# aimi-lab/robust-pose-estimator

Hardware: AMD Instinct MI355X
Metric: stereo-pair pose solves/sec (640x512, 8 solver iters) (higher is better)
Workload: dtype f32 (RAFT / geometry) + f64 (SE(3) solve), as the reference; 1 GPU; PoseNet.infer, 640x512 stereo frame pairs, 16 per GPU per step (RAFT batch 32), 12 GRU iters, lbfgs x8 SE(3) solve, weight heads on; frames_per_gpu=16, height=512, width=640, raft_iters=12, solver=lbfgs, solver_iters=8, parallelism=frames sharded x1

## Files before the change

robust-pose-estimator_amd/csrc/conv.hip:

```cpp
#include "conv_host.h"
#include "conv_igemm.h"
#include <type_traits>

template <int KW, int WM, bool ENC, int T, bool VERT, bool S2>
__global__ __launch_bounds__(256, 3) void k_conv_igemm(ConvP P) {
    constexpr int WN = 4 / WM, WT = 32 * T, BM = WT * WM, BN = WT * WN, PW = VERT ? 0 : KW / 2;
    constexpr int VTX = 16, VTY = 8, VROWS = VTY + KW - 1;
    constexpr int KS = 20;
    constexpr int NLA = BM / 64;
    constexpr int NLB = VERT ? (VROWS * VTX / 4 * CK + 255) / 256 : S2 ? BN / 32 : BN / 64;
    __shared__ __attribute__((aligned(16))) float As[2][BM][KS];
    __shared__ __attribute__((aligned(16))) float Bs[2][VERT ? VROWS * VTX : S2 ? 2 * BN + 8 : BN + 8][KS];
    const int bz = blockIdx.z, m0 = blockIdx.y * BM, n0 = blockIdx.x * BN;
    const int vtiles_x = (P.W + VTX - 1) / VTX;
    const int vx0 = VERT ? (blockIdx.x % vtiles_x) * VTX : 0, vy0 = VERT ? (blockIdx.x / vtiles_x) * VTY : 0;
    const int tid = threadIdx.x, lane = tid & 63, wv = tid >> 6, l31 = lane & 31, lh = lane >> 5;
    const int wm = wv / WN, wn = wv % WN;
    const int W = P.W, hw = P.hw, ph = P.kh / 2;
    __shared__ __attribute__((aligned(8))) float sbt[ENC ? BM : 1][2];
    if (ENC && tid < BM) {
        const int co = m0 + tid;
        sbt[tid][0] = (P.scale && co < P.cout) ? P.scale[co] : 1.0f;
        sbt[tid][1] = (P.bias && co < P.cout) ? P.bias[co] : 0.0f;
    }
// ... 304 lines not shown
#pragma unroll
                for (int r = 0; r < 4; ++r) {
                    const int row = row0 + r + 8 * (rb >> 2), co = m0 + row;
                    const bool cok = co < P.cout;
                    const float2 s2 = *(const float2*)&sbt[row][0];
                    sc[r] = s2.x; bi[r] = s2.y;
#pragma unroll
                    for (int j = 0; j < T; ++j) {
                        const int px = n0 + wn * WT + j * 32 + l31;
                        ok[j][r] = cok && px < hw;
                        e[j][r] = ok[j][r] ? (size_t)co * hw + px : 0;
                    }
                }
                if (EXTRA) {
#pragma unroll
                    for (int j = 0; j < T; ++j)
#pragma unroll
                        for (int r = 0; r < 4; ++r) {
                            rv[j][r] = resb ? resb[e[j][r]] : 0.0f;
                            av[j][r] = addb ? addb[e[j][r]] : 0.0f;
                        }
                }
#pragma unroll
                for (int r = 0; r < 4; ++r) {
                    float vv[T];
#pragma unroll
                    for (int j = 0; j < T; ++j) {
                        if (EXTRA) { float v = acc[i][j][rb + r] * sc[r]; v += av[j][r]; v += bi[r]; vv[j] = v; }
                        else vv[j] = fmaf(acc[i][j][rb + r], sc[r], bi[r]);
                    }
                    float piv[NS], ssum[NS], ssq[NS];
                    if (STATS) {
#pragma unroll
                        for (int s2 = 0; s2 < NS; ++s2) {
                            const int vb = __builtin_bit_cast(int, vv[S2 ? s2 : 0]);
                            piv[s2] = __builtin_bit_cast(float, lh ? __builtin_amdgcn_readlane(vb, 32) : __builtin_amdgcn_readlane(vb, 0));
                            ssum[s2] = 0.0f; ssq[s2] = 0.0f;
                        }
                    }
#pragma unroll
                    for (int j = 0; j < T; ++j) {
                        float v = vv[j];
                        if (STATS) { const float dv = ok[j][r] ? v - piv[S2 ? j : 0] : 0.0f; ssum[S2 ? j : 0] += dv; ssq[S2 ? j : 0] = fmaf(dv, dv, ssq[S2 ? j : 0]); }
                        if (relu) v = v < 0.0f ? 0.0f : v;
                        if (EXTRA && resb) { v = rv[j][r] + v; v = v < 0.0f ? 0.0f : v; }
                        if (ok[j][r]) { outb[e[j][r]] = v; if (EXTRA && out2b) out2b[e[j][r]] = v; }
                    }
                    if (STATS) {
                        const int row = row0 + r + 8 * (rb >> 2);
#pragma unroll
                        for (int s2 = 0; s2 < NS; ++s2) {
                            const float a = half_wave_sum(ssum[s2]), q = half_wave_sum(ssq[s2]);
                            float* rd = red + ((wn * NS + s2) * BM + row) * 3;
                            if (l31 == 31) { rd[0] = a; rd[1] = q; rd[2] = piv[s2]; }
                        }
                    }
                }
            }
        }
    };
    {
        typedef std::integral_constant<bool, true> Yes; typedef std::integral_constant<bool, false> No;
        const bool extra = P.res || P.add || P.out2;
        if (P.stats) { if (extra) epilogue(Yes{}, Yes{}); else epilogue(Yes{}, No{}); }
        else { if (extra) epilogue(No{}, Yes{}); else epilogue(No{}, No{}); }
    }
    if (P.stats) {
        __syncthreads();
        if (S2) {
            const int nrec = (hw + 31) / 32;
            if (tid < BM && m0 + tid < P.cout) {
#pragma unroll
                for (int w2 = 0; w2 < WN; ++w2)
#pragma unroll
                    for (int s2 = 0; s2 < NS; ++s2) {
                        const int blk = (n0 + w2 * WT + s2 * 32) >> 5;
                        if (blk >= nrec) continue;
                        int nw = hw - blk * 32; nw = nw > 32 ? 32 : nw;
                        const float* rd = red + ((w2 * NS + s2) * BM + tid) * 3;
                        StatAcc A;
                        A.add_pivoted(nw, rd[0], rd[1], rd[2]);
                        float* st = P.stats + (((size_t)bz * P.cout + m0 + tid) * nrec + blk) * 3;
                        st[0] = (float)A.n; st[1] = (float)A.mean; st[2] = (float)A.m2;
                    }
            }
        } else if (tid < BM && m0 + tid < P.cout) {
            StatAcc A;
#pragma unroll
            for (int w2 = 0; w2 < WN; ++w2) {
                int nw = hw - (n0 + w2 * WT); nw = nw < 0 ? 0 : (nw > WT ? WT : nw);
                A.add_pivoted(nw, red[(w2 * BM + tid) * 3], red[(w2 * BM + tid) * 3 + 1], red[(w2 * BM + tid) * 3 + 2]);
            }
            float* st = P.stats + (((size_t)bz * P.cout + m0 + tid) * gridDim.x + blockIdx.x) * 3;
            st[0] = (float)A.n; st[1] = (float)A.mean; st[2] = (float)A.m2;
        }
    }
}

__device__ __forceinline__ void plane_moments(const float* __restrict__ partials, int tiles_signed, int C, int plane, int nthreads, double* sh, double& mean, double& var) {
    const int tiles = tiles_signed < 0 ? -tiles_signed : tiles_signed;
    const int ts = tiles_signed < 0 ? 3 * C : 3;
    const float* pp = tiles_signed < 0 ? partials + ((size_t)(plane / C) * tiles * C + (plane % C)) * 3 : partials + (size_t)plane * tiles * 3;
    double n = 0.0, a = 0.0;
    for (int i = threadIdx.x; i < tiles; i += nthreads) { n += (double)pp[(size_t)ts * i]; a += (double)pp[(size_t)ts * i] * (double)pp[(size_t)ts * i + 1]; }
    n = wave_sum(n); a = wave_sum(a);
    const int nw = nthreads >> 6, wv = threadIdx.x >> 6;
    if (nw > 1) {
        if ((threadIdx.x & 63) == 0) { sh[wv] = n; sh[4 + wv] = a; }
        __syncthreads();
        n = 0.0; a = 0.0;
        for (int w = 0; w < nw; ++w) { n += sh[w]; a += sh[4 + w]; }
        __syncthreads();
    }
    mean = a / n;
    double q = 0.0;
    for (int i = threadIdx.x; i < tiles; i += nthreads) { const double d = (double)pp[(size_t)ts * i + 1] - mean; q += (double)pp[(size_t)ts * i + 2] + (double)pp[(size_t)ts * i] * d * d; }
    q = wave_sum(q);
    if (nw > 1) {
        if ((threadIdx.x & 63) == 0) sh[wv] = q;
        __syncthreads();
        q = 0.0;
        for (int w = 0; w < nw; ++w) q += sh[w];
    }
    var = q / n;
    var = var < 0.0 ? 0.0 : var;
}

__global__ __launch_bounds__(256) void k_instnorm_finalize(const float* __restrict__ partials, int tiles, int C, int hw, float eps, float* __restrict__ mi) {
    const int plane = blockIdx.x;
    __shared__ double sh[8];
    double mean, var;
    plane_moments(partials, tiles, C, plane, 256, sh, mean, var);
    if (threadIdx.x == 0) { mi[(size_t)plane * 2] = (float)mean; mi[(size_t)plane * 2 + 1] = (float)(1.0 / sqrt(var + (double)eps)); }
    (void)hw;
}

__global__ __launch_bounds__(256) void k_instnorm_finalize_tm(const float* __restrict__ partials, int tiles, int C, float eps, float* __restrict__ mi) {
    const int b = blockIdx.y, cl = threadIdx.x & 3, sl = threadIdx.x >> 2, c = blockIdx.x * 4 + cl;
    __shared__ double sh[2][64][4];
    const bool ok = c < C;
    const float* pp = partials + ((size_t)b * tiles * C + (ok ? c : 0)) * 3;
    const size_t ts = (size_t)3 * C;
    auto tree = [&](double (*v)[4]) {
#pragma unroll
        for (int h = 32; h >= 1; h >>= 1) {
            __syncthreads();
            if (sl < h) v[sl][cl] += v[sl + h][cl];
        }
        __syncthreads();
    };
    constexpr int RMAX = 20;
    float rn[RMAX], rm[RMAX], rq[RMAX];
    const bool held = tiles <= 64 * RMAX;
    if (held) {
#pragma unroll
        for (int j = 0; j < RMAX; ++j) {
            const int t = sl + 64 * j;
            const float* r = pp + ts * (size_t)(t < tiles ? t : 0);
            const float v0 = r[0], v1 = r[1], v2 = r[2];
            rn[j] = t < tiles ? v0 : 0.0f; rm[j] = v1; rq[j] = v2;
        }
    }
    double n = 0.0, a = 0.0;
    if (held) {
#pragma unroll
        for (int j = 0; j < RMAX; ++j) if (sl + 64 * j < tiles) { const double nt = (double)rn[j]; n += nt; a += nt * (double)rm[j]; }
    } else {
        for (int t = sl; t < tiles; t += 64) { const double nt = (double)pp[ts * t]; n += nt; a += nt * (double)pp[ts * t + 1]; }
    }
    sh[0][sl][cl] = n; sh[1][sl][cl] = a;
    tree(sh[0]); tree(sh[1]);
    n = sh[0][0][cl]; a = sh[1][0][cl];
    const double mean = a / n;
    double q = 0.0;
    if (held) {
#pragma unroll
        for (int j = 0; j < RMAX; ++j) if (sl + 64 * j < tiles) { const double d = (double)rm[j] - mean; q += (double)rq[j] + (double)rn[j] * d * d; }
    } else {
        for (int t = sl; t < tiles; t += 64) { const double d = (double)pp[ts * t + 1] - mean; q += (double)pp[ts * t + 2] + (double)pp[ts * t] * d * d; }
    }
    __syncthreads();
    sh[0][sl][cl] = q;
    tree(sh[0]);
    if (sl == 0 && ok) {
        double var = sh[0][0][cl] / n;
        var = var < 0.0 ? 0.0 : var;
        float* o = mi + ((size_t)b * C + c) * 2;
        o[0] = (float)mean; o[1] = (float)(1.0 / sqrt(var + (double)eps));
    }
}

__global__ __launch_bounds__(256) void k_instnorm_apply(const float* __restrict__ x, const float* __restrict__ partials, int tiles, int C, int hw,
                                                        float eps, int relu, const float* __restrict__ residual, const float* __restrict__ res_mi,
                                                        float* __restrict__ out, int split) {
    const int plane = blockIdx.x / split, part = blockIdx.x % split;
    __shared__ double sh[8];
    float mean, inv;
    if (tiles == 0) { mean = partials[(size_t)plane * 2]; inv = partials[(size_t)plane * 2 + 1]; }
    else {
        double dmean, dvar;
        plane_moments(partials, tiles, C, plane, 256, sh, dmean, dvar);
        mean = (float)dmean; inv = (float)(1.0 / sqrt(dvar + (double)eps));
    }
    const float4* xp = (const float4*)(x + (size_t)plane * hw);
    const float4* rp = residual ? (const float4*)(residual + (size_t)plane * hw) : nullptr;
    float4* op = (float4*)(out + (size_t)plane * hw);
    const bool rnorm = res_mi != nullptr;
    const float rmean = rnorm ? res_mi[(size_t)plane * 2] : 0.0f, rinv = rnorm ? res_mi[(size_t)plane * 2 + 1] : 1.0f;
    const bool yrelu = relu & 1, rrelu = !(relu & 2);
    auto fin = [&](float v, float r) -> float {
        float y = (v - mean) * inv;
        if (yrelu) y = y < 0.0f ? 0.0f : y;
        if (rp) {
            if (rnorm) { r = (r - rmean) * rinv; if (rrelu) r = r < 0.0f ? 0.0f : r; }
            y = r + y; y = y < 0.0f ? 0.0f : y;
        }
        return y;
    };
#ifndef INA_UNROLL
#define INA_UNROLL 4
#endif
#ifndef INA_NT
#define INA_NT 3
#endif
    typedef float f4 __attribute__((ext_vector_type(4)));
    const int n4all = hw >> 2;
    const int per = ((n4all + split - 1) / split + 3) & ~3;
    const int n4 = (part + 1) * per < n4all ? (part + 1) * per : n4all;
    int i = part * per + threadIdx.x;
    for (; i + (INA_UNROLL - 1) * (int)blockDim.x < n4; i += INA_UNROLL * blockDim.x) {
        f4 v[INA_UNROLL], r[INA_UNROLL];
#pragma unroll
        for (int u = 0; u < INA_UNROLL; ++u) {
            const int j = i + u * blockDim.x;
            v[u] = INA_NT ? __builtin_nontemporal_load((const f4*)xp + j) : ((const f4*)xp)[j];
            r[u] = rp ? (INA_NT ? __builtin_nontemporal_load((const f4*)rp + j) : ((const f4*)rp)[j]) : (f4){0.f, 0.f, 0.f, 0.f};
        }
#pragma unroll
        for (int u = 0; u < INA_UNROLL; ++u) {
            const f4 o = {fin(v[u][0], r[u][0]), fin(v[u][1], r[u][1]), fin(v[u][2], r[u][2]), fin(v[u][3], r[u][3])};
            if (INA_NT & 2) __builtin_nontemporal_store(o, (f4*)op + i + u * blockDim.x); else ((f4*)op)[i + u * blockDim.x] = o;
        }
    }
    for (; i < n4; i += blockDim.x) {
        const float4 v = xp[i];
        const float4 r = rp ? rp[i] : make_float4(0.f, 0.f, 0.f, 0.f);
        op[i] = make_float4(fin(v.x, r.x), fin(v.y, r.y), fin(v.z, r.z), fin(v.w, r.w));
    }
}

__global__ void k_conv_pack(const float* __restrict__ w, float* __restrict__ wp, int cout, int cin, int kh, int kw, int coP,
                            long long total) {
    const long long e = (long long)blockIdx.x * blockDim.x + threadIdx.x;
    if (e >= total) return;
    const int ke = (int)(e & 3);
    const int co = (int)((e >> 2) % coP);
    const long long rest = (e >> 2) / coP;
    const int k4 = (int)(rest & 3);
    const long long s = rest >> 2;
    const int dx = (int)(s % kw), dy = (int)((s / kw) % kh), c = (int)(s / ((long long)kw * kh));
    const int ci = c * CK + 4 * k4 + ke;
    wp[e] = (co < cout && ci < cin) ? w[(((size_t)co * cin + ci) * kh + dy) * kw + dx] : 0.0f;
}

static inline bool conv_wide(int cout) { return (cout % 128) != 0 && (cout % 128) <= 96; }
static inline bool conv_s2_small(int cout, int hw_out, int b) { return (long long)ceil_div(hw_out, 128) * ceil_div(cout, 128) * b < 512; }

extern "C" size_t rpe_conv_packed_floats(int cout, int cin, int kh, int kw) {
    if (cout <= 0 || cin <= 0 || kh <= 0 || kw <= 0) return 0;
    return ((size_t)((cin + CK - 1) / CK) * kh * kw + 1) * CK * round_up(cout, 128);
}

extern "C" int rpe_conv_pack(const float* weight, int cout, int cin, int kh, int kw, float* packed, void* stream) {
    if (kh <= 0 || kw <= 0) return RPE_E_BADARG;
    return launch_pack(k_conv_pack, weight, packed, cout, cin, 1, (long long)rpe_conv_packed_floats(cout, cin, kh, kw), stream, kh, kw, round_up(cout, 128));
}

static_assert(sizeof(rpe_conv_desc) == 200, "rpe_conv_desc layout is part of the ABI (ctypes mirror in _lib.py)");

static int conv_fused(const rpe_conv_desc* d, void* stream, bool m96) {
    if (!conv_desc_present(d)) return RPE_E_BADARG;
    if (d->kh < 1 || !(d->kh & 1) || (d->kw != 1 && d->kw != 3 && d->kw != 5)) return RPE_E_UNSUPPORTED;
    if ((d->w & 3) || !aligned16(d->x, d->x_batch_stride)) return RPE_E_UNSUPPORTED;
    if (d->mode < RPE_CONV_LINEAR || d->mode > RPE_CONV_TANH) return RPE_E_BADARG;
    if (d->mode == RPE_CONV_TANH && (!conv_no_encoder_epilogue(d) || !stride_is_1(d) ||
                                     ((d->cout % 64) != 0 && (d->cout % 64) <= 32 && d->kw == 3))) return RPE_E_UNSUPPORTED;
    if (!conv_gate_args_ok(d)) return RPE_E_BADARG;
    if ((d->mode == RPE_CONV_GATE_ZR || d->mode == RPE_CONV_GATE_H) && (d->scale || d->residual || d->stats)) return RPE_E_BADARG;
    const int stride = d->stride ? d->stride : 1;
    if (stride != 1 && stride != 2) return RPE_E_UNSUPPORTED;
    if (d->pre_norm && (stride != 1 || d->kw != 3 || d->mode > RPE_CONV_RELU)) return RPE_E_UNSUPPORTED;
    if (stride == 2 && ((d->h & 1) || (d->w & 1) || d->mode > RPE_CONV_RELU || !((d->kh == 3 && d->kw == 3) || (d->kh == 1 && d->kw == 1))))
        return RPE_E_UNSUPPORTED;
    ConvP P;
    fill_common(P, d, round_up(d->cout, 128)); fill_gate(P, d); fill_encoder(P, d);
    P.kh = d->kh; P.Hin = d->h; P.Win = d->w; P.H = d->h / stride; P.W = d->w / stride; P.hw = P.H * P.W;
    P.h = d->hidden; P.hbs = d->hidden_batch_stride;
    hipStream_t s = (hipStream_t)stream;
    if (stride == 2) {
        const int t128 = ceil_div(P.hw, 128), t64 = ceil_div(P.hw, 64);
        const bool small = conv_s2_small(d->cout, P.hw, d->b);
        if (d->stats && d->stats_tiles != 0 && d->stats_tiles != ceil_div(P.hw, 32)) return RPE_E_BADARG;
        if (m96 && d->kw == 3 && d->cout == 96 && !d->residual && !d->add && !d->out2) return conv_s2_m96_launch(P, d->b, s);
        if (small) {
            dim3 g2(t64, ceil_div(d->cout, 64), d->b);
            if (d->kw == 3) hipLaunchKernelGGL((k_conv_igemm<3, 2, true, 1, false, true>), g2, dim3(256), 0, s, P);
            else hipLaunchKernelGGL((k_conv_igemm<1, 2, true, 1, false, true>), g2, dim3(256), 0, s, P);
            return rpe_check_launch();
        }
        dim3 g2(t128, ceil_div(d->cout, 128), d->b);
        if (d->kw == 3) hipLaunchKernelGGL((k_conv_igemm<3, 2, true, 2, false, true>), g2, dim3(256), 0, s, P);
        else hipLaunchKernelGGL((k_conv_igemm<1, 2, true, 2, false, true>), g2, dim3(256), 0, s, P);
        return rpe_check_launch();
    }
    bool wide = conv_wide(d->cout);
    int BM = wide ? 64 : 128, BN = wide ? 256 : 128;
    const bool half_tile = (d->cout % 64) != 0 && (d->cout % 64) <= 32 && d->kw == 3 && d->mode <= RPE_CONV_RELU;
    const bool enc = d->scale || d->residual || d->stats || d->pre_norm || half_tile;
    const bool small = !enc && (long long)ceil_div(P.hw, BN) * ceil_div(d->cout, BM) * d->b < 512;
    if (small) { BM = 64; BN = 64; }
    dim3 grid(ceil_div(P.hw, BN), ceil_div(d->cout, BM), d->b), block(256);
#define LAUNCH(KW_, WM_, ENC_, T_) hipLaunchKernelGGL((k_conv_igemm<KW_, WM_, ENC_, T_, false, false>), grid, block, 0, s, P)
    if (enc) {
        if (d->kw != 3 || d->mode > RPE_CONV_RELU) return RPE_E_UNSUPPORTED;
        if (wide) LAUNCH(3, 1, true, 2); else LAUNCH(3, 2, true, 2);
    } else if (small) { if (d->kw == 1) LAUNCH(1, 2, false, 1); else if (d->kw == 3) LAUNCH(3, 2, false, 1); else LAUNCH(5, 2, false, 1); }
    else if (wide) { if (d->kw == 1) LAUNCH(1, 1, false, 2); else if (d->kw == 3) LAUNCH(3, 1, false, 2); else LAUNCH(5, 1, false, 2); }
    else if (d->kw == 1 && d->kh == 5) {
        dim3 vgrid(ceil_div(d->w, 16) * ceil_div(d->h, 8), grid.y, grid.z);
        hipLaunchKernelGGL((k_conv_igemm<5, 2, false, 2, true, false>), vgrid, block, 0, s, P);
    } else         { if (d->kw == 1) LAUNCH(1, 2, false, 2); else if (d->kw == 3) LAUNCH(3, 2, false, 2); else LAUNCH(5, 2, false, 2); }
#undef LAUNCH
    return rpe_check_launch();
}

extern "C" int rpe_conv_fused(const rpe_conv_desc* d, void* stream) { return conv_fused(d, stream, false); }
extern "C" int rpe_conv_fused_m96(const rpe_conv_desc* d, void* stream) { return conv_fused(d, stream, true); }

extern "C" int rpe_conv_stats_tiles(int cout, int h, int w, int stride) {
    if (cout <= 0 || h <= 0 || w <= 0 || (stride != 1 && stride != 2)) return 0;
    if (stride == 2) return ceil_div((int64_t)(h / 2) * (w / 2), 32);
    return ceil_div((int64_t)h * w, conv_wide(cout) ? 256 : 128);
}

extern "C" int rpe_conv_stats_tiles_batch(int cout, int h, int w, int stride, int b) {
    if (b <= 0) return 0;
    return rpe_conv_stats_tiles(cout, h, w, stride);
}

extern "C" int rpe_instnorm_apply_ex(const float* x, const float* partials, int tiles, int b, int c, int hw, float eps, int relu,
                                     const float* residual, const float* residual_mean_inv, float* out, void* stream) {
    if (!x || !partials || !out || b <= 0 || c <= 0 || hw <= 0 || (residual_mean_inv && !residual)) return RPE_E_BADARG;
    if ((hw & 3) || !aligned16(x, 0) || !aligned16(out, 0) || !aligned16(residual, 0)) return RPE_E_UNSUPPORTED;
    int split = 1;
#ifndef INA_MAXSPLIT
#define INA_MAXSPLIT 16
#endif
#ifndef INA_MINBYTES
#define INA_MINBYTES 16384
#endif
    if (tiles == 0) while (split < INA_MAXSPLIT && (long long)hw * 4 / (split * 2) >= INA_MINBYTES) split *= 2;
    hipLaunchKernelGGL(k_instnorm_apply, dim3(b * c * split), dim3(256), 0, (hipStream_t)stream, x, partials, tiles, c, hw, eps, relu, residual,
                       residual_mean_inv, out, split);
    return rpe_check_launch();
}

extern "C" int rpe_instnorm_apply(const float* x, const float* partials, int tiles, int b, int c, int hw, float eps, int relu,
                                  const float* residual, float* out, void* stream) {
    return rpe_instnorm_apply_ex(x, partials, tiles, b, c, hw, eps, relu, residual, nullptr, out, stream);
}

extern "C" int rpe_instnorm_finalize(const float* partials, int tiles, int b, int c, int hw, float eps, float* mean_inv, void* stream) {
    if (!partials || !mean_inv || tiles == 0 || b <= 0 || c <= 0 || hw <= 0) return RPE_E_BADARG;
    if (tiles < 0) hipLaunchKernelGGL(k_instnorm_finalize_tm, dim3(ceil_div(c, 4), b), dim3(256), 0, (hipStream_t)stream, partials, -tiles, c, eps, mean_inv);
    else hipLaunchKernelGGL(k_instnorm_finalize, dim3(b * c), dim3(256), 0, (hipStream_t)stream, partials, tiles, c, hw, eps, mean_inv);
    return rpe_check_launch();
}
```

robust-pose-estimator_amd/csrc/conv_igemm.h:

```cpp
#pragma once
#include "rpe_common.h"

typedef float f32x16 __attribute__((ext_vector_type(16)));
#define CK 16
#define SCHED_FENCE() __builtin_amdgcn_sched_barrier(0)

struct ConvP {
    const float* x; long long xbs;
    const float* wp;
    int cin, cout, coP, H, W, hw, kh;
    int Hin, Win;
    const float* bias;
    const float* add; long long abs_;
    int mode;
    float* out; long long obs;
    float* out2; long long o2bs;
    const float* h; long long hbs;
    const float* z; long long zbs;
    int cgate;
    const float* scale;
    const float* res; long long rbs;
    float* stats;
    const float* pre;
};


__device__ __forceinline__ float half_wave_sum(float v) {
    v += __builtin_bit_cast(float, __builtin_amdgcn_update_dpp(0, __builtin_bit_cast(int, v), 0xB1, 0xF, 0xF, true));
    v += __builtin_bit_cast(float, __builtin_amdgcn_update_dpp(0, __builtin_bit_cast(int, v), 0x4E, 0xF, 0xF, true));
    v += __builtin_bit_cast(float, __builtin_amdgcn_update_dpp(0, __builtin_bit_cast(int, v), 0x141, 0xF, 0xF, true));
    v += __builtin_bit_cast(float, __builtin_amdgcn_update_dpp(0, __builtin_bit_cast(int, v), 0x140, 0xF, 0xF, true));
    v += __builtin_bit_cast(float, __builtin_amdgcn_update_dpp(0, __builtin_bit_cast(int, v), 0x142, 0xA, 0xF, true));
    return v;
}

int conv_s2_m96_launch(const ConvP& P, int batch, hipStream_t stream);
```

robust-pose-estimator_amd/raft.py:

```python
import operator
from types import SimpleNamespace

import torch
import torch.nn as nn

from . import ops

WINOGRAD = True
WINO_2X4 = True
S2_M96 = True
S2_M96_MIN_WGS = 512
CORR_BF16X3 = False
CONV_BF16X3 = False
X3_MIN_CIN = 128
X3_GRU = False
SIDE_STREAM = True
PAD_MAPS = False
LOOP_OPLIST = True
LOOKUP_EVENT_SINK = None
FRAME_OPLISTS = True
LOOKUP_FUSED = True
LOOKUP_FUSED_MAX_WGS = 256
FRAME_OPLISTS_MAX_IMAGES = 4
ENC_STREAMS = True
ENC_STREAMS_MIN = 8
SIDE_STREAM_MAX = 8 * 5120
ROUTE_SWITCHES = ('WINOGRAD', 'WINO_2X4', 'S2_M96', 'S2_M96_MIN_WGS', 'CORR_BF16X3', 'CONV_BF16X3', 'X3_MIN_CIN', 'X3_GRU', 'SIDE_STREAM', 'SIDE_STREAM_MAX',
                  'LOOKUP_FUSED', 'LOOKUP_FUSED_MAX_WGS', 'ENC_STREAMS', 'ENC_STREAMS_MIN', 'PAD_MAPS')
_switch_values = operator.itemgetter(*ROUTE_SWITCHES)


def _switches():
    return _switch_values(globals())


def padded_size(h8, w8):
    return h8 + (h8 & 1), (w8 + 3) // 4 * 4


def _norm(kind, ch):
    if kind == 'batch':
        return nn.BatchNorm2d(ch)
    if kind == 'instance':
        return nn.InstanceNorm2d(ch)
    if kind == 'none':
        return nn.Sequential()
    raise ValueError(kind)


class ResidualBlock(nn.Module):
    def __init__(self, in_planes, planes, norm_fn='batch', stride=1):
        super().__init__()
        self.conv1 = nn.Conv2d(in_planes, planes, kernel_size=3, padding=1, stride=stride)
        self.conv2 = nn.Conv2d(planes, planes, kernel_size=3, padding=1)
        self.relu = nn.ReLU(inplace=True)
        self.norm1 = _norm(norm_fn, planes)
        self.norm2 = _norm(norm_fn, planes)
        if stride == 1:
            self.downsample = None
        else:
            self.norm3 = _norm(norm_fn, planes)
            self.downsample = nn.Sequential(nn.Conv2d(in_planes, planes, kernel_size=1, stride=stride), self.norm3)

    def takes_raw_input(self, x):
        return (isinstance(self.norm1, nn.InstanceNorm2d) and self.downsample is None and _fusable(self.conv1, x) and x.shape[-1] % 4 == 0
                and _wino(self.conv1, x) is not None)

    def forward(self, x, x_norm=None):
        fused_in = isinstance(self.norm1, nn.InstanceNorm2d) and _fusable(self.conv1, x) and x.shape[-1] // self.conv1.stride[0] % 4 == 0
        if x_norm is not None and not (fused_in and self.takes_raw_input(x)):
            raise RuntimeError('ResidualBlock: x_norm needs the fused stride-1 Winograd route')
        if fused_in:
            st = self.conv1.stride[0]
            hw = (x.shape[-2] // st) * (x.shape[-1] // st)
            raw1, stats1 = _encoder_conv(self.conv1, x, pre_norm=x_norm, moments=True)
            mi = ops.instnorm_finalize(stats1, hw, eps=self.norm1.eps, channels=self.conv1.out_channels)
            res_relu = True
            if self.downsample is not None:
                sc = self.downsample[0]
                if _fusable(sc, x):
                    x, stats_sc = _encoder_conv(sc, x, moments=True)
                    x_norm = ops.instnorm_finalize(stats_sc, hw, eps=self.norm3.eps, channels=sc.out_channels)
                    res_relu = False
                else:
                    x = conv_norm_act(sc, self.norm3, x, relu=False)
            raw2, stats2 = _encoder_conv(self.conv2, raw1, pre_norm=mi, moments=True)
            if isinstance(stats2, ops.TileMajorStats):
                stats2 = ops.instnorm_finalize(stats2, hw, eps=self.norm2.eps, channels=self.conv2.out_channels)
            return ops.instnorm_apply(raw2, stats2, eps=self.norm2.eps, relu=True, residual=x, residual_norm=x_norm, residual_relu=res_relu)
        y = conv_norm_act(self.conv1, self.norm1, x, relu=True)
        if self.downsample is not None:
            x = conv_norm_act(self.downsample[0], self.norm3, x, relu=False)
        return conv_norm_act(self.conv2, self.norm2, y, relu=True, residual=x)


def _bounded_put(cache, key, value, keep=2):
    while len(cache) >= keep:
        cache.pop(next(iter(cache)))
    cache[key] = value


def _wkey(*tensors):
    return tuple(None if t is None else (t._version, t.data_ptr()) for t in tensors)


def _cached(owner, attr, key, make, with_key=False):
    d = owner if isinstance(owner, dict) else owner.__dict__
    cached = d.get(attr)
    if cached is None or cached[0] != key:
        d[attr] = cached = (key, make())
    return cached if with_key else cached[1]


def _bn_affine(conv, norm):
    def fold():
        scale = (norm.weight / torch.sqrt(norm.running_var + norm.eps)).detach().float().contiguous()
        return scale, ((conv.bias - norm.running_mean) * scale + norm.bias).detach().float().contiguous()
    return _cached(norm, '_rpe_affine', _wkey(conv.bias, norm.weight, norm.bias, norm.running_mean, norm.running_var), fold)


def _packed(conv):
    return _cached(conv, '_rpe_packed', _wkey(conv.weight), lambda: ops.PackedConv(conv.weight, None))


def _wino(conv, x):
    if not WINOGRAD or conv.stride != (1, 1) or conv.kernel_size != (3, 3) or conv.padding != (1, 1):
        return None
    if not ops.PackedWino.supported(conv.weight, x.shape[-2], x.shape[-1]) or conv.in_channels > 128 or not x.is_contiguous():
        return None
    kind = ops.PackedWino24 if WINO_2X4 and ops.PackedWino24.supported(conv.weight, x.shape[-2], x.shape[-1]) else ops.PackedWino
    return _cached(conv, '_rpe_wino', (_wkey(conv.weight), kind), lambda: kind(conv.weight, None))


def _fusable(conv, x):
    _, _, hh, ww = x.shape
    s1 = conv.stride == (1, 1) and conv.kernel_size == (3, 3) and conv.padding == (1, 1)
    s2 = conv.stride == (2, 2) and hh % 2 == 0 and ww % 2 == 0 and \
        ((conv.kernel_size == (3, 3) and conv.padding == (1, 1)) or (conv.kernel_size == (1, 1) and conv.padding == (0, 0)))
    stride = 2 if s2 else 1
    return (s1 or s2) and ww % 4 == 0 and ((hh // stride) * (ww // stride)) % 4 == 0 and x.is_contiguous()


def conv_norm_act(conv, norm, x, relu, residual=None):
    fused = _fusable(conv, x)
    if isinstance(norm, nn.BatchNorm2d):
        if norm.training:
            raise RuntimeError('the RAFT encoders run with frozen batch norm (RAFT.freeze_bn, pose_net.py:22)')
        scale, shift = _bn_affine(conv, norm)
        if fused:
            return _encoder_conv(conv, x, ops.CONV_RELU if relu else ops.CONV_LINEAR, affine=(scale, shift), residual=residual)[0]
        return ops.affine_act(ops.conv_direct(x, conv.weight, None, conv.stride, conv.padding), scale, shift, relu=relu, residual=residual)
    if isinstance(norm, nn.InstanceNorm2d):
        if fused:
            pre, stats = _encoder_conv(conv, x, moments=True)
            return ops.instnorm_apply(pre, stats, eps=norm.eps, relu=relu, residual=residual)
        return ops.instnorm_act(ops.conv_direct(x, conv.weight, None, conv.stride, conv.padding), conv.bias, eps=norm.eps, relu=relu, residual=residual)
    raise NotImplementedError(type(norm))


def _encoder_conv(conv, x, mode=ops.CONV_LINEAR, affine=None, residual=None, pre_norm=None, moments=False):
    b, _, hh, ww = x.shape
    st, cout = conv.stride[0], conv.out_channels
    scale, bias = affine if affine is not None else (None, conv.bias.detach())
    pw = _wino(conv, x)
    out = torch.empty(b, cout, hh // st, ww // st, device=x.device)
    if pw is not None:
        stats = ops.conv_wino_stats_buffer(b, cout, hh, ww, x.device) if moments else None
        ops.conv_wino(x, pw, mode, out, scale=scale, bias=bias, residual=residual, stats=stats, pre_norm=pre_norm)
    else:
        stats = ops.conv_stats_buffer(b, cout, hh, ww, x.device, stride=st) if moments else None
        m96 = S2_M96 and st == 2 and conv.kernel_size == (3, 3) and cout == 96 and b * -(-(hh // 2) * (ww // 2) // 128) >= S2_M96_MIN_WGS
        ops.conv_fused(x, _packed(conv), mode, out, scale=scale, bias=bias, residual=residual, stats=stats, stride=st, pre_norm=pre_norm,
                       entry='rpe_conv_fused_m96' if m96 else 'rpe_conv_fused')
    return out, stats


def _recording(owner, root):
    d = owner.__dict__
    if d.get('_recorded') is None:
        d['_recorded'] = _Recorded()
    if '_key_tensors' not in d:
        d['_key_tensors'] = [(slots, n) for m in root.modules() for slots in (m._parameters, m._buffers) for n in slots]
    return d['_recorded'], _wkey(*[slots[n] for slots, n in d['_key_tensors']])


def _overlap(tensors):
    spans = sorted((t.data_ptr(), t.data_ptr() + t.numel() * t.element_size()) for t in tensors)
    return any(a[1] > b[0] for a, b in zip(spans, spans[1:]))


class _Recorded:

    def __init__(self, keep=4):
        self._progs, self._failed, self._keep = {}, {}, keep

    def get(self, key):
        return self._progs.get(key)

    def wanted(self, key):
        return self._failed.get(key, 0) < 3

    def put(self, key, rec):
        if rec.complete:
            _bounded_put(self._progs, key, rec, keep=self._keep)
        else:
            if len(self._failed) > 64:
                self._failed.clear()
            self._failed[key] = self._failed.get(key, 0) + 1

    def clear(self):
        self._progs.clear()
        self._failed.clear()


class BasicEncoder(nn.Module):
    def __init__(self, output_dim=128, norm_fn='batch', dropout=0.0):
        super().__init__()
        self.norm_fn = norm_fn
        self.norm1 = _norm(norm_fn, 64)
        self.conv1 = nn.Conv2d(3, 64, kernel_size=7, stride=2, padding=3)
        self.relu1 = nn.ReLU(inplace=True)
        self.in_planes = 64
        self.layer1 = self._make_layer(64, stride=1)
        self.layer2 = self._make_layer(96, stride=2)
        self.layer3 = self._make_layer(128, stride=2)
        self.conv2 = nn.Conv2d(128, output_dim, kernel_size=1)
        for m in self.modules():
            if isinstance(m, nn.Conv2d):
                nn.init.kaiming_normal_(m.weight, mode='fan_out', nonlinearity='relu')
            elif isinstance(m, (nn.BatchNorm2d, nn.InstanceNorm2d)):
                if m.weight is not None:
                    nn.init.constant_(m.weight, 1)
                if m.bias is not None:
                    nn.init.constant_(m.bias, 0)

    def _make_layer(self, dim, stride=1):
        l1 = ResidualBlock(self.in_planes, dim, self.norm_fn, stride=stride)
        l2 = ResidualBlock(dim, dim, self.norm_fn, stride=1)
        self.in_planes = dim
        return nn.Sequential(l1, l2)

    def _stem_pack(self):
        w = self.conv1.weight
        return _cached(self, '_stem_packed', _wkey(w), lambda: ops.PackedStem(w))

    def _stem_many(self, images):
        ps = self._stem_pack()
        n = sum(im.shape[0] for im in images)
        hh, ww = images[0].shape[-2:]
        out = torch.empty(n, 64, hh // 2, ww // 2, device=images[0].device)
        bn = isinstance(self.norm1, nn.BatchNorm2d)
        if bn:
            if self.norm1.training:
                raise RuntimeError('the RAFT encoders run with frozen batch norm (RAFT.freeze_bn, pose_net.py:22)')
            scale, shift = _bn_affine(self.conv1, self.norm1)
        stats = None if bn else torch.empty(n, 64, ops.lib().rpe_stem_tiles(hh, ww, 2), 3, device=out.device)
        i = 0
        for im in images:
            k = im.shape[0]
            if bn:
                ops.stem_conv(im.contiguous(), ps, bias=shift, scale=scale, relu=True, out=out[i:i + k])
            else:
                ops.stem_conv(im.contiguous(), ps, bias=self.conv1.bias.detach(), relu=False, stats=stats[i:i + k], out=out[i:i + k])
            i += k
        if bn:
            return out, None
        if self.layer1[0].takes_raw_input(out):
            return out, ops.instnorm_finalize(stats, (hh // 2) * (ww // 2), eps=self.norm1.eps, channels=64)
        return ops.instnorm_apply(out, stats, eps=self.norm1.eps, relu=True), None

    def _final(self, x, split_act):
        m = self.conv2
        b, _, hh, ww = x.shape
        half = m.out_channels // 2
        if ww % 4 == 0 and x.is_contiguous():
            def pack():
                w, bv = m.weight.detach(), m.bias.detach()
                return ops.Conv1x1(w, bv), ops.Conv1x1(w[:half].contiguous(), bv[:half].contiguous()), ops.Conv1x1(w[half:].contiguous(), bv[half:].contiguous())
            whole, lo, hi = _cached(self, '_final_packed', _wkey(m.weight, m.bias), pack)
            out = torch.empty(b, m.out_channels, hh, ww, device=x.device)
            if not split_act:
                return whole(x, ops.CONV_LINEAR, out, x3=CONV_BF16X3)
            lo(x, ops.CONV_TANH, out[:, :half])
            hi(x, ops.CONV_RELU, out[:, half:], x3=CONV_BF16X3)
            return out
        y = ops.conv_direct(x, m.weight, m.bias, 1, 0)
        if split_act:
            y[:, :half] = torch.tanh(y[:, :half])
            ops.bias_act(y[:, half:].contiguous(), None, relu=True, out=y, out_offset=half)
        return y

    def _apply(self, fn, *a, **k):
        r = super()._apply(fn, *a, **k)
        self.__dict__.pop('_key_tensors', None)
        if getattr(self, '_recorded', None) is not None:
            self._recorded.clear()
        return r

    def forward(self, x, raw255=False, split_act=False):
        images = list(x) if isinstance(x, (list, tuple)) else [x]
        first = images[0]
        if FRAME_OPLISTS and raw255 and first.is_cuda and first.device.index == torch.cuda.current_device() and not torch.is_grad_enabled() \
                and sum(im.shape[0] for im in images) <= FRAME_OPLISTS_MAX_IMAGES \
                and all(im.is_contiguous() and im.dtype == torch.float32 and im.device == first.device for im in images) and not _overlap(images):
            recorded, wkey = _recording(self, self)
            key = (tuple(tuple(im.shape) for im in images), first.device.index, ops.raw_stream(), split_act, _switches(), self.training, wkey)
            rec = recorded.get(key)
            if rec is not None:
                out = torch.empty(rec.out_shape, device=first.device)
                rec.replay({**{i: im for i, im in enumerate(images)}, 'out': out})
                return out
            if recorded.wanted(key):
                rec = ops.Recorder()
                with rec:
                    out = self._forward(x, raw255, split_act)
                if rec.complete and out.is_contiguous():
                    for i, im in enumerate(images):
                        rec.complete = rec.complete and rec.bind(i, im) > 0
                    rec.complete = rec.complete and rec.bind('out', out) > 0
                    rec.out_shape = tuple(out.shape)
                recorded.put(key, rec)
                return out
        return self._forward(x, raw255, split_act)

    def _forward(self, x, raw255=False, split_act=False):
        many = isinstance(x, (list, tuple))
        first = x[0] if many else x
        hh, ww = first.shape[-2:]
        stem_ok = raw255 and hh % 2 == 0 and ww % 2 == 0 and ((hh // 2) * (ww // 2)) % 4 == 0 and isinstance(self.norm1, (nn.BatchNorm2d, nn.InstanceNorm2d))
        x_norm = None
        if stem_ok:
            x, x_norm = self._stem_many(list(x) if many else [x])
        else:
            x = (torch.cat(list(x), dim=0) if many else x).contiguous()
            x = conv_norm_act(self.conv1, self.norm1, 2 * (x / 255.0) - 1.0 if raw255 else x, relu=True)
        x = self.layer1[1](self.layer1[0](x, x_norm))
        x = self.layer3(self.layer2(x))
        return self._final(x, split_act)


class FlowHead(nn.Module):
    def __init__(self, input_dim=128, hidden_dim=256):
        super().__init__()
        self.conv1 = nn.Conv2d(input_dim, hidden_dim, 3, padding=1)
        self.conv2 = nn.Conv2d(hidden_dim, 2, 3, padding=1)
        self.relu = nn.ReLU(inplace=True)

    def forward(self, x):
        return self.conv2(self.relu(self.conv1(x)))


class SepConvGRU(nn.Module):

    def __init__(self, hidden_dim=128, input_dim=192 + 128):
        super().__init__()
        c = hidden_dim + input_dim
        self.convz1 = nn.Conv2d(c, hidden_dim, (1, 5), padding=(0, 2))
        self.convr1 = nn.Conv2d(c, hidden_dim, (1, 5), padding=(0, 2))
        self.convq1 = nn.Conv2d(c, hidden_dim, (1, 5), padding=(0, 2))
        self.convz2 = nn.Conv2d(c, hidden_dim, (5, 1), padding=(2, 0))
        self.convr2 = nn.Conv2d(c, hidden_dim, (5, 1), padding=(2, 0))
        self.convq2 = nn.Conv2d(c, hidden_dim, (5, 1), padding=(2, 0))


class BasicMotionEncoder(nn.Module):
    def __init__(self, corr_levels=4, corr_radius=4):
        super().__init__()
        cor_planes = corr_levels * (2 * corr_radius + 1) ** 2
        self.convc1 = nn.Conv2d(cor_planes, 256, 1, padding=0)
        self.convc2 = nn.Conv2d(256, 192, 3, padding=1)
        self.convf1 = nn.Conv2d(2, 128, 7, padding=3)
        self.convf2 = nn.Conv2d(128, 64, 3, padding=1)
        self.conv = nn.Conv2d(64 + 192, 128 - 2, 3, padding=1)

    def flow_branch(self, flow, P, L):
        ops.stem_conv(flow, P['convf1'], bias=self.convf1.bias.detach(), relu=True, div=1.0, mul=1.0, sub=0.0, out=L.flo, **L.vk)
        L.f2()

    def forward(self, flow, corr, cat_buf, hx, rhx):
        def cv(m, x):
            return ops.conv_direct(x, m.weight, None, m.stride, m.padding)
        cor = ops.bias_act(cv(self.convc1, corr), self.convc1.bias)
        ops.bias_act(cv(self.convc2, cor), self.convc2.bias, out=cat_buf, out_offset=0)
        flo = ops.bias_act(cv(self.convf1, flow), self.convf1.bias)
        ops.bias_act(cv(self.convf2, flo), self.convf2.bias, out=cat_buf, out_offset=192)
        ops.bias_act(cv(self.conv, cat_buf), self.conv.bias, out=hx, out_offset=128, out2=rhx, out2_offset=128)
        ops.bias_act(flow, None, relu=False, out=hx, out_offset=254, out2=rhx, out2_offset=254)


class BasicUpdateBlock(nn.Module):
    def __init__(self, corr_levels=4, corr_radius=4, hidden_dim=128):
        super().__init__()
        self.hidden_dim = hidden_dim
        self.encoder = BasicMotionEncoder(corr_levels, corr_radius)
        self.gru = SepConvGRU(hidden_dim=hidden_dim, input_dim=128 + hidden_dim)
        self.flow_head = FlowHead(hidden_dim, hidden_dim=256)
        self.mask = nn.Sequential(nn.Conv2d(128, 256, 3, padding=1), nn.ReLU(inplace=True),
                                  nn.Conv2d(256, 64 * 9, 1, padding=0))

    def gate_weights(self, with_key=False):
        g, c = self.gru, self.hidden_dim

        def split(w):
            return torch.cat((w[:, :c], w[:, 2 * c:]), 1).detach().contiguous(), w[:, c:2 * c].detach().contiguous()

        def stack():
            W = {}
            for name, convs in (('zr1', (g.convz1, g.convr1)), ('q1', (g.convq1,)), ('zr2', (g.convz2, g.convr2)), ('q2', (g.convq2,))):
                w = torch.cat([m.weight for m in convs], 0)
                bvec = torch.cat([m.bias for m in convs], 0).detach().contiguous()
                W[name] = (*split(w), bvec)
            return W
        key = _wkey(*[t for m in (g.convz1, g.convr1, g.convq1, g.convz2, g.convr2, g.convq2) for t in (m.weight, m.bias)])
        return _cached(self, '_stacked', key, stack, with_key)

    def context_terms(self, inp, out=None):
        W = self.gate_weights()
        P = self.packed_convs(inp.shape[-1]) if out is not None else None
        if P is not None:
            for k in W:
                (ops.conv_wino1d if isinstance(P['ctx_' + k], ops.PackedWino1d) else ops.conv_fused)(inp, P['ctx_' + k], ops.CONV_LINEAR, out[k])
            return out
        pads = {'zr1': (0, 2), 'q1': (0, 2), 'zr2': (2, 0), 'q2': (2, 0)}
        return {k: ops.conv_direct(inp, W[k][1], W[k][2], 1, pads[k]) for k in W}

    def packed_convs(self, width, with_key=False):
        if width % 4 != 0:
            return (None, None) if with_key else None
        e, fh = self.encoder, self.flow_head
        mods = (e.convc1, e.convc2, e.convf2, e.conv, fh.conv1)
        gate_key, W = self.gate_weights(with_key=True)
        key = (_wkey(*[t for m in mods + (e.convf1,) for t in (m.weight, m.bias)]), gate_key, _switches())
        return _cached(self, '_packed', key, lambda: self._pack_convs(mods, W), with_key)

    def _pack_convs(self, mods, W):
        e = self.encoder
        P = {n: ops.PackedConv(m.weight, m.bias) for n, m in zip(('convc1', 'convc2', 'convf2', 'conv', 'fh1'), mods)}
        P['wino'] = {n: ops.PackedWino(m.weight, m.bias) for n, m in zip(('convc2', 'convf2', 'conv', 'fh1'), mods[1:])
                     if ops.PackedWino.supported(m.weight, 2, 2)} if WINOGRAD else {}
        P['wino24'] = {n: ops.PackedWino24(m.weight, m.bias) for n, m in zip(('convc2', 'convf2', 'conv', 'fh1'), mods[1:])
                       if ops.PackedWino24.supported(m.weight, 2, 4)} if (WINOGRAD and WINO_2X4 and not CONV_BF16X3) else {}
        P['wino_x3'] = {n: ops.PackedWinoX3(m.weight, m.bias) for n, m in zip(('convc2', 'convf2', 'conv', 'fh1'), mods[1:])
                        if n != 'convf2' and m.in_channels >= X3_MIN_CIN and ops.PackedWinoX3.supported(m.weight, 2, 4)} if (WINOGRAD and CONV_BF16X3) else {}
        P['convf1'] = ops.PackedStem(e.convf1.weight)
        P['convc1_1x1'] = ops.Conv1x1(e.convc1.weight, e.convc1.bias)
        for n in ('zr1', 'q1', 'zr2', 'q2'):
            P[n] = (ops.PackedWino1dX3 if CONV_BF16X3 and X3_GRU and ops.PackedWino1dX3.supported(W[n][0], 4) else ops.PackedWino1d)(W[n][0]) if WINOGRAD \
                else ops.PackedConv(W[n][0])
            P['ctx_' + n] = (ops.PackedWino1d if WINOGRAD else ops.PackedConv)(W[n][1], W[n][2])
        scratch = {}

        def buf(name, like, c):
            k = (name, like.data_ptr(), like.shape[0], c, like.shape[2], like.shape[3], like.device)
            if k not in scratch:
                _bounded_put(scratch, k, torch.empty(like.shape[0], c, like.shape[2], like.shape[3], device=like.device), keep=12)
            return scratch[k]
        P['cor_buf'] = lambda like: buf('cor', like, 256)
        P['fh_buf'] = lambda like: buf('fh', like, 256)
        P['flo_buf'] = lambda like: buf('flo', like, 128)
        return P

    def launchers(self, ws, pyr=None, with_key=False):
        packed_key, P = self.packed_convs(ws['hx'].shape[-1], with_key=True)
        alt = isinstance(pyr, ops.AltCorr)
        key = (packed_key, None if pyr is None else (pyr.buf.data_ptr(), alt), ws.get('valid'))
        return _cached(ws, '_launchers', key, lambda: self._make_launchers(ws, P, pyr, alt), with_key)

    def _make_launchers(self, ws, P, pyr, alt):
        hx, rhx, z_buf, cat_buf, corr, coords1, flow, ctx = (ws[k] for k in ('hx', 'rhx', 'z', 'cat', 'corr', 'coords1', 'flow', 'ctx'))
        c = self.hidden_dim
        e, fh = self.encoder, self.flow_head
        cor, flo, fh_buf = P['cor_buf'](corr), P['flo_buf'](corr), P['fh_buf'](hx)
        valid = ws.get('valid')
        vk = {} if valid is None else dict(valid=valid)
        wino = dict(P['wino']) if hx.shape[-1] % 2 == 0 and hx.shape[-2] % 2 == 0 else {}
        if wino and hx.shape[-1] % 4 == 0:
# ... 415 lines not shown
```

Baseline: 251.5 pose solves/s.

## Add specialized stride-2 1x1 conv kernel for encoder downsample projections

Adds a dedicated MFMA kernel for stride-2 1x1 convolutions with (cin,cout) of (64,96) or (96,128). It preloads all weights into shared memory once, uses a tile that covers every output channel, and double-buffers the input tiles, with a fused affine/ReLU/statistics epilogue. It is routed through the m96 entry whenever there are enough workgroups. The aim is to replace the generic implicit-GEMM path for the encoder's downsample shortcut convs. The cost is more code paths and higher shared-memory use per block.

After: 252.1 pose solves/s, median of 6. No clear change (+0.2%).

```diff
diff --git a/robust-pose-estimator_amd/csrc/conv.hip b/robust-pose-estimator_amd/csrc/conv.hip
--- a/robust-pose-estimator_amd/csrc/conv.hip
+++ b/robust-pose-estimator_amd/csrc/conv.hip
@@ -630,6 +630,7 @@
         const bool small = conv_s2_small(d->cout, P.hw, d->b);
         if (d->stats && d->stats_tiles != 0 && d->stats_tiles != ceil_div(P.hw, 32)) return RPE_E_BADARG;
         if (m96 && d->kw == 3 && d->cout == 96 && !d->residual && !d->add && !d->out2) return conv_s2_m96_launch(P, d->b, s);
+        if (m96 && d->kw == 1 && conv1x1_s2_takes(d->cin, d->cout) && !d->residual && !d->add && !d->out2) return conv1x1_s2_launch(P, d->b, s);
         if (small) {
             dim3 g2(t64, ceil_div(d->cout, 64), d->b);
             if (d->kw == 3) hipLaunchKernelGGL((k_conv_igemm<3, 2, true, 1, false, true>), g2, dim3(256), 0, s, P);
diff --git a/robust-pose-estimator_amd/csrc/conv1x1_s2.hip b/robust-pose-estimator_amd/csrc/conv1x1_s2.hip
--- /dev/null
+++ b/robust-pose-estimator_amd/csrc/conv1x1_s2.hip
@@ -0,0 +1,156 @@
+#include "conv_igemm.h"
+#include <type_traits>
+
+template <int NB, int NCH>
+__global__ __launch_bounds__(256, 2) void k_conv1x1_s2(ConvP P) {
+    constexpr int BM = 32 * NB, BN = 128, KS = 20, NLB = BN / 32;
+    __shared__ __attribute__((aligned(16))) float As[NCH][BM][KS];
+    __shared__ __attribute__((aligned(16))) float Bs[2][BN][KS];
+    const int bz = blockIdx.z, n0 = blockIdx.x * BN;
+    const int tid = threadIdx.x, lane = tid & 63, wv = tid >> 6, l31 = lane & 31, lh = lane >> 5;
+    const int W = P.W, hw = P.hw;
+    const int sb_m = tid < BM ? tid : 0;
+    float sb_s = 1.0f, sb_b = 0.0f;
+    if (P.scale) sb_s = P.scale[sb_m];
+    if (P.bias) sb_b = P.bias[sb_m];
+    const size_t hw_in = (size_t)P.Hin * P.Win;
+    const int i1 = 256 + (BM == 128 ? tid : (tid & 127));
+    const int a_m0 = tid % BM, a_k40 = tid / BM, a_m1 = i1 % BM, a_k41 = i1 / BM;
+    const float* w0 = P.wp + ((size_t)a_k40 * P.coP + a_m0) * 4;
+    const float* w1 = P.wp + ((size_t)a_k41 * P.coP + a_m1) * 4;
+    const size_t wstep = (size_t)4 * P.coP * 4;
+    float4 wa0[NCH], wa1[NCH];
+#pragma unroll
+    for (int c = 0; c < NCH; ++c) { wa0[c] = *(const float4*)(w0 + c * wstep); wa1[c] = *(const float4*)(w1 + c * wstep); }
+    const int b_k = (tid >> 2) & 15, b_n4 = (tid & 3) + 4 * wv;
+    const float* xrow = P.x + (size_t)bz * P.xbs + (size_t)b_k * hw_in;
+    const float* src[NLB];
+    unsigned ok = 0;
+#pragma unroll
+    for (int u = 0; u < NLB; ++u) {
+        const int na = n0 + 2 * (b_n4 + 16 * u);
+        const int y = na / W, x = na - y * W;
+        const bool o = na < hw;
+        src[u] = o ? xrow + (size_t)(2 * y) * P.Win + 2 * x : P.x;
+        ok |= o ? (1u << u) : 0u;
+    }
+    float4 rb[NCH][NLB];
+#pragma unroll
+    for (int c = 0; c < NCH; ++c)
+#pragma unroll
+        for (int u = 0; u < NLB; ++u) rb[c][u] = *(const float4*)(src[u] + (size_t)c * CK * hw_in);
+    const bool odd_tap = P.kh != 1;
+#pragma unroll
+    for (int c = 0; c < NCH; ++c) {
+        *(float4*)&As[c][a_m0][4 * a_k40] = wa0[c];
+        *(float4*)&As[c][a_m1][4 * a_k41] = wa1[c];
+    }
+    *(float2*)&As[0][sb_m][16] = make_float2(sb_s, sb_b);
+
+    f32x16 acc[NB];
+#pragma unroll
+    for (int i = 0; i < NB; ++i)
+#pragma unroll
+        for (int r = 0; r < 16; ++r) acc[i][r] = 0.0f;
+
+    typedef float f32x4 __attribute__((ext_vector_type(4)));
+    f32x4 ah1[NB], ah2[NB], bh1, bh2;
+#define S2X1_STORE_B(c, buf)                                                                                             \
+    _Pragma("unroll") for (int u = 0; u < NLB; ++u) {                                                                    \
+        const int n = 2 * (b_n4 + 16 * u);                                                                               \
+        const bool o = (ok >> u) & 1;                                                                                    \
+        const float e0 = odd_tap ? rb[c][u].y : rb[c][u].x, e1 = odd_tap ? rb[c][u].w : rb[c][u].z;                      \
+        Bs[buf][n][b_k] = o ? e0 : 0.0f; Bs[buf][n + 1][b_k] = o ? e1 : 0.0f;                                            \
+    }
+#define S2X1_READ(ah, bh, c, buf, half)                                                                                  \
+    {                                                                                                                    \
+        const float* arow = &As[c][l31][8 * lh + 4 * (half)];                                                            \
+        _Pragma("unroll") for (int i = 0; i < NB; ++i) ah[i] = *(const f32x4*)(arow + 32 * i * KS);                      \
+        bh = *(const f32x4*)&Bs[buf][wv * 32 + l31][8 * lh + 4 * (half)];                                                \
+    }
+#define S2X1_MMA(ah, bh)                                                                                                 \
+    _Pragma("unroll") for (int j = 0; j < 4; ++j)                                                                        \
+        _Pragma("unroll") for (int i = 0; i < NB; ++i)                                                                   \
+            acc[i] = __builtin_amdgcn_mfma_f32_32x32x2f32(ah[i][j], bh[j], acc[i], 0, 0, 0);
+
+    S2X1_STORE_B(0, 0)
+    __syncthreads();
+    S2X1_READ(ah1, bh1, 0, 0, 0)
+#pragma unroll
+    for (int c = 0; c < NCH; ++c) {
+        const int cur = c & 1;
+        S2X1_READ(ah2, bh2, c, cur, 1)
+        SCHED_FENCE();
+        S2X1_MMA(ah1, bh1)
+        SCHED_FENCE();
+        if (c + 1 < NCH) { S2X1_STORE_B(c + 1, cur ^ 1) }
+        __syncthreads();
+        if (c + 1 < NCH) S2X1_READ(ah1, bh1, c + 1, cur ^ 1, 0)
+        SCHED_FENCE();
+        S2X1_MMA(ah2, bh2)
+        SCHED_FENCE();
+    }
+#undef S2X1_STORE_B
+#undef S2X1_READ
+#undef S2X1_MMA
+
+    float* red = &As[1][0][0];
+    static_assert(4 * 3 <= (NCH - 1) * KS, "statistics scratch must fit the weights tiles behind the first");
+    const int px = n0 + wv * 32 + l31;
+    const bool pok = px < hw;
+    float* outb = P.out + (size_t)bz * P.obs;
+    const bool relu = P.mode == RPE_CONV_RELU;
+    auto epilogue = [&](auto statsc) {
+        constexpr bool STATS = decltype(statsc)::value;
+#pragma unroll
+        for (int i = 0; i < NB; ++i) {
+            const int row0 = i * 32 + 4 * lh;
+#pragma unroll
+            for (int rb4 = 0; rb4 < 16; rb4 += 4) {
+#pragma unroll
+                for (int r = 0; r < 4; ++r) {
+                    const int row = row0 + r + 8 * (rb4 >> 2);
+                    const float2 s2 = *(const float2*)&As[0][row][16];
+                    float v = fmaf(acc[i][rb4 + r], s2.x, s2.y);
+                    if (STATS) {
+                        const int vb = __builtin_bit_cast(int, v);
+                        const float piv = __builtin_bit_cast(float, lh ? __builtin_amdgcn_readlane(vb, 32) : __builtin_amdgcn_readlane(vb, 0));
+                        const float dv = pok ? v - piv : 0.0f;
+                        float ssum = 0.0f, ssq = 0.0f;
+                        ssum += dv; ssq = fmaf(dv, dv, ssq);
+                        const float a = half_wave_sum(ssum), q = half_wave_sum(ssq);
+                        float* rd = red + (wv * BM + row) * 3;
+                        if (l31 == 31) { rd[0] = a; rd[1] = q; rd[2] = piv; }
+                    }
+                    if (relu) v = v < 0.0f ? 0.0f : v;
+                    if (pok) outb[(size_t)row * hw + px] = v;
+                }
+            }
+        }
+    };
+    if (P.stats) epilogue(std::integral_constant<bool, true>{}); else epilogue(std::integral_constant<bool, false>{});
+    if (P.stats) {
+        __syncthreads();
+        const int nrec = (hw + 31) / 32;
+        if (tid < BM) {
+#pragma unroll
+            for (int w2 = 0; w2 < 4; ++w2) {
+                const int blk = (n0 + w2 * 32) >> 5;
+                if (blk >= nrec) continue;
+                int nw = hw - blk * 32; nw = nw > 32 ? 32 : nw;
+                const float* rd = red + (w2 * BM + tid) * 3;
+                StatAcc A;
+                A.add_pivoted(nw, rd[0], rd[1], rd[2]);
+                float* st = P.stats + (((size_t)bz * P.cout + tid) * nrec + blk) * 3;
+                st[0] = (float)A.n; st[1] = (float)A.mean; st[2] = (float)A.m2;
+            }
+        }
+    }
+}
+
+int conv1x1_s2_launch(const ConvP& P, int batch, hipStream_t stream) {
+    const dim3 grid(ceil_div(P.hw, 128), 1, batch);
+    if (P.cout == 96) hipLaunchKernelGGL((k_conv1x1_s2<3, 4>), grid, dim3(256), 0, stream, P);
+    else hipLaunchKernelGGL((k_conv1x1_s2<4, 6>), grid, dim3(256), 0, stream, P);
+    return rpe_check_launch();
+}
diff --git a/robust-pose-estimator_amd/csrc/conv_igemm.h b/robust-pose-estimator_amd/csrc/conv_igemm.h
--- a/robust-pose-estimator_amd/csrc/conv_igemm.h
+++ b/robust-pose-estimator_amd/csrc/conv_igemm.h
@@ -35,3 +35,5 @@
 }
 
 int conv_s2_m96_launch(const ConvP& P, int batch, hipStream_t stream);
+static inline bool conv1x1_s2_takes(int cin, int cout) { return (cin == 64 && cout == 96) || (cin == 96 && cout == 128); }
+int conv1x1_s2_launch(const ConvP& P, int batch, hipStream_t stream);
diff --git a/robust-pose-estimator_amd/raft.py b/robust-pose-estimator_amd/raft.py
--- a/robust-pose-estimator_amd/raft.py
+++ b/robust-pose-estimator_amd/raft.py
@@ -10,6 +10,8 @@
 WINO_2X4 = True
 S2_M96 = True
 S2_M96_MIN_WGS = 512
+S2X1 = True
+S2X1_MIN_WGS = 512
 CORR_BF16X3 = False
 CONV_BF16X3 = False
 X3_MIN_CIN = 128
@@ -25,7 +27,7 @@
 ENC_STREAMS = True
 ENC_STREAMS_MIN = 8
 SIDE_STREAM_MAX = 8 * 5120
-ROUTE_SWITCHES = ('WINOGRAD', 'WINO_2X4', 'S2_M96', 'S2_M96_MIN_WGS', 'CORR_BF16X3', 'CONV_BF16X3', 'X3_MIN_CIN', 'X3_GRU', 'SIDE_STREAM', 'SIDE_STREAM_MAX',
+ROUTE_SWITCHES = ('WINOGRAD', 'WINO_2X4', 'S2_M96', 'S2_M96_MIN_WGS', 'S2X1', 'S2X1_MIN_WGS', 'CORR_BF16X3', 'CONV_BF16X3', 'X3_MIN_CIN', 'X3_GRU', 'SIDE_STREAM', 'SIDE_STREAM_MAX',
                   'LOOKUP_FUSED', 'LOOKUP_FUSED_MAX_WGS', 'ENC_STREAMS', 'ENC_STREAMS_MIN', 'PAD_MAPS')
 _switch_values = operator.itemgetter(*ROUTE_SWITCHES)
 
@@ -169,9 +171,12 @@
         ops.conv_wino(x, pw, mode, out, scale=scale, bias=bias, residual=residual, stats=stats, pre_norm=pre_norm)
     else:
         stats = ops.conv_stats_buffer(b, cout, hh, ww, x.device, stride=st) if moments else None
-        m96 = S2_M96 and st == 2 and conv.kernel_size == (3, 3) and cout == 96 and b * -(-(hh // 2) * (ww // 2) // 128) >= S2_M96_MIN_WGS
+        wgs = b * -(-(hh // 2) * (ww // 2) // 128)
+        m96 = S2_M96 and st == 2 and conv.kernel_size == (3, 3) and cout == 96 and wgs >= S2_M96_MIN_WGS
+        s2x1 = S2X1 and st == 2 and conv.kernel_size == (1, 1) and (conv.in_channels, cout) in ((64, 96), (96, 128)) and residual is None \
+            and wgs >= S2X1_MIN_WGS
         ops.conv_fused(x, _packed(conv), mode, out, scale=scale, bias=bias, residual=residual, stats=stats, stride=st, pre_norm=pre_norm,
-                       entry='rpe_conv_fused_m96' if m96 else 'rpe_conv_fused')
+                       entry='rpe_conv_fused_m96' if m96 or s2x1 else 'rpe_conv_fused')
     return out, stats
 
 
```
